# ziyaad30/ForwardTacotron

Hardware: AMD Instinct MI355X
Metric: mel_frames_per_sec_train_step (higher is better)
Workload: dtype f32

## Files before the change

### forwardtacotron_amd/csrc/ft_capi_core.hip

```cpp
#include <stdarg.h>
#include <stdio.h>
#include <string.h>

#include "../../include/fwdtaco_hip.h"
#include <mutex>
#include <utility>
#include <vector>

#include "ft_gemm.h"

static thread_local char g_err[512] = "";

void ft_set_error(const char* fmt, ...) {
  va_list ap;
  va_start(ap, fmt);
  vsnprintf(g_err, sizeof(g_err), fmt, ap);
  va_end(ap);
}

int ft_check_launch(const char* what) {
  hipError_t e = hipGetLastError();
  if (e != hipSuccess) {
    ft_set_error("%s: HIP launch failed: %s", what, hipGetErrorString(e));
    return FT_ERR_HIP;
// ... 455 lines not shown
static int conv1d_bwd_data_impl(const float* dy, long lddy, const float* wp, float* dx, long lddx, int B, int T, int Cin,
                                int Cout, int k, int Tbuf, int Tvalid, int accumulate, int wp_transposed,
                                const float* relu_mask, void* stream) {
  FT_REQUIRE(k >= 1 && Tvalid <= Tbuf, "conv1d_bwd_data: bad k/Tvalid");
  FtGemmBatch b;
  memset(&b, 0, sizeof(b));
  b.relu_mask = relu_mask;
  FtGemmTask& t = b.t[0];
  t.A = dy; t.B = wp; t.C = dx;
  t.lda = lddy; t.ldb = wp_transposed ? Cout : Cin; t.ldc = lddx; t.b_tap_stride = (long)Cout * Cin;
  t.M = B * T; t.N = Cin; t.K = Cout; t.taps = k;
  FtRowMap m = {T > 0 ? T : 1, Tbuf, 1, Tvalid, k / 2, -1};
  t.amap = m;
  t.accumulate = accumulate;
  return ft_launch_gemm_rows(&b, 1, !wp_transposed, (hipStream_t)stream);
}

static bool bank_bwd_partials(int B, int T, int Cin, int K) {
  const long tiles = (long)ft_cdiv((long)B * T, 128) * ft_cdiv(Cin, 128);
  return K >= 2 && Cin > 64 && (long)B * T > 64 && tiles < 192 && tiles * K >= 192;
}

size_t ft_conv_bank_bwd_data_workspace(int B, int T, int Cin, int K) {
  return bank_bwd_partials(B, T, Cin, K) ? (size_t)K * B * T * Cin * sizeof(float) : 0;
}

int ft_conv_bank_bwd_data(const float* dy, long lddy, const float* wp_all, float* dx, long lddx, int B, int T, int Cin,
                          int C, int K, int Tbuf, int wp_transposed, void* workspace, size_t workspace_bytes,
                          void* stream) {
  FT_REQUIRE(K >= 1 && K <= FT_MAX_TASKS, "conv_bank_bwd_data: K=%d unsupported (max %d)", K, FT_MAX_TASKS);
  FT_REQUIRE(Tbuf == T || Tbuf == T + 1, "conv_bank_bwd_data: Tbuf must be T or T+1");
  const bool partials = bank_bwd_partials(B, T, Cin, K);
  if (partials)
    FT_REQUIRE(workspace && workspace_bytes >= ft_conv_bank_bwd_data_workspace(B, T, Cin, K),
               "conv_bank_bwd_data: workspace too small");
  float* part = static_cast<float*>(workspace);
  FtGemmBatch b;
  memset(&b, 0, sizeof(b));
  long woff = 0;
  for (int i = 0; i < K; ++i) {
    const int k = i + 1;
    FtGemmTask& t = b.t[i];
    t.A = dy + (long)i * C; t.B = wp_all + woff;
    t.C = partials ? part + (long)i * B * T * Cin : dx;
    t.lda = lddy; t.ldb = wp_transposed ? C : Cin; t.ldc = partials ? Cin : lddx; t.b_tap_stride = (long)C * Cin;
    t.M = B * T; t.N = Cin; t.K = C; t.taps = k;
    const int Tvalid = (k % 2 == 0) ? Tbuf : T;
    FtRowMap m = {T > 0 ? T : 1, Tbuf, 1, Tvalid < Tbuf ? Tvalid : Tbuf, k / 2, -1};
    t.amap = m;
    woff += (long)k * C * Cin;
  }
  b.chain = partials ? 0 : K;
  if (partials && wp_transposed) {
    FtGemmBatch c = b;
    for (int i = 0; i < K; ++i) {
      c.t[i].C = dx;
      c.t[i].ldc = lddx;
    }
    c.chain = K;
    const size_t need = ft_rows_ksplit_floats(c, K, (hipStream_t)stream) * sizeof(float);
    if (need > 0 && need <= workspace_bytes) {
      c.ksplit_slab = part;
      return ft_launch_gemm_rows(&c, K, false, (hipStream_t)stream);
    }
  }
  int rc = ft_launch_gemm_rows(&b, K, !wp_transposed, (hipStream_t)stream);
  if (rc || !partials) return rc;
  return ft_launch_slab_sum(part, dx, B * T, Cin, K, lddx, (hipStream_t)stream);
}

static FtGemmTNTask conv_bw_task(const float* dy, long lddy, const float* x, long ldx, float* dw, int B, int T,
                                 int Cin, int Cout, int k, int Tbuf, int Tvalid) {
  FtGemmTNTask t;
  memset(&t, 0, sizeof(t));
  t.A = dy; t.B = x; t.dst = dw;
  t.lda = lddy; t.ldb = ldx;
// ... 151 lines not shown
```

### forwardtacotron_amd/csrc/ft_gemm.h

```cpp
#pragma once
#include "ft_common.h"

struct FtRowMap {
  int Tlog, bstride, tstride, Tvalid, shift0, shift_step;
};

static inline FtRowMap ft_rowmap_identity(int rows) {
  int n = rows > 0 ? rows : 1;
  FtRowMap m = {n, 0, 1, n, 0, 0};
  return m;
}
static inline FtRowMap ft_rowmap_layout(int rows, int tm_B) {
  if (tm_B <= 0) return ft_rowmap_identity(rows);
  int T = rows / tm_B;
  FtRowMap m = {T > 0 ? T : 1, 1, tm_B, T, 0, 0};
  return m;
}

struct FtGemmTask {
  const float* A;
  const float* B;
  float* C;
  const float* bias;
  const float* scale;
// ... 145 lines not shown
    int kk = 1, first = 0;
    while (first + kk <= q) {
      first += kk;
      ++kk;
    }
    w.kk = kk;
    w.zts = q - first;
    w.mtile = (kk - 1) * tpm + sub;
    w.s = blockIdx.z;
  } else {
    w.kk = 0;
    w.mtile = blockIdx.x;
    w.zts = blockIdx.z / S;
    w.s = blockIdx.z - w.zts * S;
  }
  return w;
}

static inline bool ft_rows_tile_is_big(long tiles128, int maxM, int maxN) { return tiles128 >= 192 && maxN > 64 && maxM > 64; }
static_assert(sizeof(FtGemmBatch) <= 4080, "FtGemmBatch travels as a kernel argument (4 KB limit)");
int ft_launch_gemm_rows(FtGemmBatch* batch, int ntasks, bool b_ncontig, hipStream_t stream);
size_t ft_rows_ksplit_floats(const FtGemmBatch& batch, int ntasks, hipStream_t stream);
int ft_launch_ksplit_reduce(const float* slab, int S, const FtGemmTask& t, hipStream_t stream);
bool ft_rows_b3p_ok(const FtGemmBatch& batch, int ntask);
int ft_launch_gemm_rows_b3(const FtGemmBatch& batch, bool big, dim3 grid, hipStream_t stream);
int ft_launch_gemm_tn_b3(const FtGemmTNTask& t, float* slab, int S, int rows_per_split, int tm, dim3 grid,
                         hipStream_t stream);
void ft_note_stream_slots(hipStream_t s, int slots);
int ft_stream_slots(hipStream_t s);
bool ft_gemm_b3_enabled();
int ft_gemm_precision();
int ft_launch_gemm_tn(const FtGemmTNTask& task, float* workspace, size_t workspace_floats,
                      hipStream_t stream);
size_t ft_gemm_tn_workspace_floats(const FtGemmTNTask& task);
int ft_launch_slab_sum(const float* slab, float* dst, int M, int N, int S, long ldm, hipStream_t stream);
```

### forwardtacotron_amd/csrc/ft_gemm.hip

```cpp
#include "ft_gemm.h"

namespace {

constexpr int BK = 32;

__device__ __forceinline__ float4 ld4(const float* p, int remaining, bool vec) {
  float4 v = make_float4(0.f, 0.f, 0.f, 0.f);
  if (remaining >= 4 && vec) {
    v = *reinterpret_cast<const float4*>(p);
  } else {
    if (remaining > 0) v.x = p[0];
    if (remaining > 1) v.y = p[1];
    if (remaining > 2) v.z = p[2];
    if (remaining > 3) v.w = p[3];
  }
  return v;
}

template <int TM, int TN, int LDA, int LDB>
__device__ __forceinline__ void mfma_stage(const float* ap, const float* bp, f32x16 (&acc)[TM][TN]) {
  float a0[TM], b0[TN], a1[TM], b1[TN];
#pragma unroll
  for (int i = 0; i < TM; ++i) a0[i] = ap[32 * i];
#pragma unroll
// ... 582 lines not shown
static int rows_ksplit_plan(const FtGemmBatch& b, int ntasks, hipStream_t stream) {
  static const bool enabled = [] {
    const char* e = getenv("FT_GEMM_KSPLIT");
    return !(e && e[0] == '0');
  }();
  const bool chained = b.chain > 1;
  if (!enabled || !(chained ? b.chain == ntasks : ntasks == 1) || !ft_gemm_b3_enabled()) return 1;
  const FtGemmTask& t0 = b.t[0];
  if (t0.nz > 1 || t0.relu || t0.scale || t0.stat || b.hw_mode || b.relu_mask || t0.N % 4 != 0 || t0.M <= 64 || t0.N <= 64) return 1;
  if (!ft_rows_b3p_ok(b, ntasks)) return 1;
  long stages = 0;
  for (int i = 0; i < ntasks; ++i) stages += (long)b.t[i].taps * ft_cdiv(b.t[i].K, 16);
  const long tiles = (long)ft_cdiv(t0.M, 128) * ft_cdiv(t0.N, 128);
  const long slots = ft_stream_slots(stream);
  if (stages < 128) return 1;
  long S = slots / (tiles > 0 ? tiles : 1);
  if (S > stages / 32) S = stages / 32;
  if (S > 16) S = 16;
  if (S < 2) return 1;
  const long per = (stages + S - 1) / S;
  return (int)((stages + per - 1) / per);
}

size_t ft_rows_ksplit_floats(const FtGemmBatch& batch, int ntasks, hipStream_t stream) {
  const int S = rows_ksplit_plan(batch, ntasks, stream);
  return S > 1 ? (size_t)S * batch.t[0].M * batch.t[0].N : 0;
}

int ft_launch_gemm_rows(FtGemmBatch* batch, int ntasks, bool b_ncontig, hipStream_t stream) {
  FT_REQUIRE(ntasks >= 1 && ntasks <= FT_MAX_TASKS, "gemm_rows: bad task count %d", ntasks);
  int maxM = 0, maxN = 0;
  long tiles128 = 0;
  for (int i = 0; i < ntasks; ++i) {
    FtGemmTask& t = batch->t[i];
    FT_REQUIRE(t.M >= 0 && t.N >= 0 && t.K >= 0 && t.taps >= 1, "gemm_rows: bad dims");
    FT_REQUIRE(t.amap.Tlog > 0, "gemm_rows: bad row map");
    if (t.cmap.Tlog <= 0) t.cmap = ft_rowmap_identity(t.M);
    if (t.nz <= 1) {
      t.nz = t.nz1 = 1;
      t.sA0 = t.sA1 = t.sB0 = t.sB1 = t.sC0 = t.sC1 = 0;
    }
    FT_REQUIRE(t.nz == 1 || ntasks == 1, "gemm_rows: strided batch needs a single task");
    FT_REQUIRE(t.nz1 >= 1 && t.nz % t.nz1 == 0, "gemm_rows: bad batch split");
    t.a_vec = (t.lda % 4 == 0) && (((uintptr_t)t.A) % 16 == 0) && (t.sA0 % 4 == 0) && (t.sA1 % 4 == 0);
    t.b_vec = (t.ldb % 4 == 0) && (t.b_tap_stride % 4 == 0) && (((uintptr_t)t.B) % 16 == 0) && (t.sB0 % 4 == 0) &&
              (t.sB1 % 4 == 0);
    if (t.M > maxM) maxM = t.M;
    if (t.N > maxN) maxN = t.N;
    tiles128 += (long)ft_cdiv(t.M, 128) * ft_cdiv(t.N, 128) * t.nz;
  }
  if (maxM == 0 || maxN == 0) return FT_OK;
  for (int i = ntasks; i < FT_MAX_TASKS; ++i) batch->t[i] = batch->t[0];
  const bool chained = batch->chain > 1;
  if (chained) {
    FT_REQUIRE(batch->chain == ntasks, "gemm_rows: chain must cover all tasks");
    for (int i = 0; i < ntasks; ++i)
      FT_REQUIRE(batch->t[i].M == batch->t[0].M && batch->t[i].N == batch->t[0].N && batch->t[i].nz == 1,
                 "gemm_rows: chained tasks must share M and N");
    tiles128 /= ntasks;
  } else {
    batch->chain = 0;
  }
  bool big = batch->force_tile ? batch->force_tile == 2 : ft_rows_tile_is_big(tiles128, maxM, maxN);
  batch->ksplit = 0;
  if (batch->ksplit_slab) {
    bool ok = !b_ncontig && ft_gemm_precision() == 0;
    for (int i = 0; i < ntasks && ok; ++i) {
      const FtGemmTask& t = batch->t[i];
      ok = (t.lda % 4 == 0) && (((uintptr_t)t.A) % 16 == 0) && (t.ldb % 4 == 0) && (t.b_tap_stride % 4 == 0) &&
           (((uintptr_t)t.B) % 16 == 0) && t.K % 4 == 0;
    }
    const int S = ok ? rows_ksplit_plan(*batch, ntasks, stream) : 1;
    if (S > 1) {
      batch->ksplit = S;
      big = true;
    }
  }
  const int bm = big ? 128 : 64;
  dim3 grid(ft_cdiv(maxM, bm), ft_cdiv(maxN, bm), chained ? 1 : (ntasks == 1 ? batch->t[0].nz : ntasks));
  if (batch->ksplit > 1) grid.z = batch->ksplit;
  FT_REQUIRE(grid.y <= 65535 && grid.z <= 65535, "gemm_rows: grid too large");
  bool fast = true;
  for (int i = 0; i < ntasks; ++i) {
    const FtGemmTask& t = batch->t[i];
    const bool k_ok = t.K % 4 == 0 || (b_ncontig && t.a_rowpad && t.lda >= ((t.K + 3) & ~3));
    fast = fast && t.a_vec && t.b_vec && k_ok && (!b_ncontig || t.N % 4 == 0);
  }
#define FT_ROWS_LAUNCH(TM_, BNC_)                                                                              \
  do {                                                                                                         \
    if (fast)                                                                                                  \
      hipLaunchKernelGGL((ft_gemm_rows_kernel<TM_, TM_, BNC_, true>), grid, dim3(256), 0, stream, *batch);     \
    else                                                                                                       \
      hipLaunchKernelGGL((ft_gemm_rows_kernel<TM_, TM_, BNC_, false>), grid, dim3(256), 0, stream, *batch);    \
  } while (0)
  GemmLog log;
  log.begin(stream);
  const bool b3 = fast && !b_ncontig && ((big && ft_gemm_b3_enabled()) || ft_gemm_precision() == 1);
  batch->stat_fused = b3 && big && !chained;
  if (b3) {
    (void)ft_launch_gemm_rows_b3(*batch, big, grid, stream);
  } else if (big) {
    if (b_ncontig) FT_ROWS_LAUNCH(2, true);
    else FT_ROWS_LAUNCH(2, false);
  } else {
    if (b_ncontig) FT_ROWS_LAUNCH(1, true);
    else FT_ROWS_LAUNCH(1, false);
  }
#undef FT_ROWS_LAUNCH
  if (GemmLog::on()) {
    double fl = 0;
    long sk = 0;
    for (int i = 0; i < ntasks; ++i) {
      const FtGemmTask& t = batch->t[i];
      fl += 2.0 * t.M * t.N * t.K * t.taps * t.nz;
      sk += (long)t.K * t.taps;
    }
    log.end(b_ncontig ? "rowsNN" : (b3 ? (ft_gemm_precision() == 1 ? "rowsBF" : "rowsB3") : "rowsNT"), maxM, maxN, sk, ntasks, batch->t[0].nz,
            big ? "128" : "64", fl);
  }
  int rc = ft_check_launch("gemm_rows");
  if (rc == FT_OK && batch->ksplit > 1) rc = ft_launch_ksplit_reduce(batch->ksplit_slab, batch->ksplit, batch->t[0], stream);
  return rc;
}

int ft_launch_slab_sum(const float* slab, float* dst, int M, int N, int S, long ldm, hipStream_t stream) {
  long total = (long)M * N;
  if (total == 0) return FT_OK;
  hipLaunchKernelGGL(ft_splitk_reduce_kernel, dim3(ft_cdiv(total, 256)), dim3(256), 0, stream, slab, dst, M, N, 1, S,
                     ldm, 1L, 0L, 0, 1, 1, 0L, 0L);
  return ft_check_launch("slab_sum");
}

int ft_launch_gemm_tn(const FtGemmTNTask& task_in, float* workspace, size_t workspace_floats,
                      hipStream_t stream) {
  FtGemmTNTask t = task_in;
  FT_REQUIRE(t.M >= 0 && t.N >= 0 && t.R >= 0 && t.taps >= 1, "gemm_tn: bad dims");
  if (t.M == 0 || t.N == 0) return FT_OK;
  if (t.nz <= 1) {
    t.nz = t.nz1 = 1;
    t.sA0 = t.sA1 = t.sB0 = t.sB1 = t.sD0 = t.sD1 = 0;
  }
// ... 62 lines not shown
```

### forwardtacotron_amd/csrc/ft_gemm_b3.hip

```cpp
#include "ft_gemm.h"
#include "ft_split.h"

namespace {

constexpr int BK = 32;
constexpr int RS = 104;

typedef __bf16 bf16x8 __attribute__((ext_vector_type(8)));
typedef unsigned short u16x4 __attribute__((ext_vector_type(4)));
typedef unsigned u32x4 __attribute__((ext_vector_type(4)));

__device__ __forceinline__ float4 ld4_sel(const float* p, const float* safe, bool ok) {
  const float4 v = *reinterpret_cast<const float4*>(ok ? p : safe);
  return ok ? v : make_float4(0.f, 0.f, 0.f, 0.f);
}

__device__ __forceinline__ unsigned rn_pack(float a, float b) { return ft_rn_pack(a, b); }
__device__ __forceinline__ void split_pair(float a, float b, unsigned& hi, unsigned& mid, unsigned& lo) {
  ft_split_pair(a, b, hi, mid, lo);
}
__device__ __forceinline__ void split3(const float4& v, u16x4& hi, u16x4& mid, u16x4& lo) {
  unsigned h[2], m[2], l[2];
  split_pair(v.x, v.y, h[0], m[0], l[0]);
  split_pair(v.z, v.w, h[1], m[1], l[1]);
  hi = __builtin_bit_cast(u16x4, uint2{h[0], h[1]});
  mid = __builtin_bit_cast(u16x4, uint2{m[0], m[1]});
  lo = __builtin_bit_cast(u16x4, uint2{l[0], l[1]});
}

__device__ __forceinline__ void store_split(unsigned short* row, const float4& v) {
  u16x4 h, m, l;
  split3(v, h, m, l);
  *reinterpret_cast<u16x4*>(row) = h;
  *reinterpret_cast<u16x4*>(row + 32) = m;
  *reinterpret_cast<u16x4*>(row + 64) = l;
}

__device__ __forceinline__ void store_rn(unsigned short* row, const float4& v) {
  typedef __bf16 bf16x4 __attribute__((ext_vector_type(4)));
  bf16x4 r = {(__bf16)v.x, (__bf16)v.y, (__bf16)v.z, (__bf16)v.w};
  *reinterpret_cast<bf16x4*>(row) = r;
}

template <int TM, int TN>
__device__ __forceinline__ void rows_b3_epilogue(const FtGemmTask& T, float* TC, f32x16 (&acc)[TM][TN], unsigned short* smem,
                                                 int m0, int n0, int tM, int tN, int tid, int mtile,
                                                 const float* relu_mask = nullptr) {
  const int wave = tid >> 6, lane = tid & 63;
  const int wm = wave >> 1, wn = wave & 1;
  const int half = lane >> 5, l31 = lane & 31;
  const float* ebias = T.bias;
  const float* escale = T.scale;
  const float* eshift = T.shift;
  const bool erelu = T.relu != 0, eacc = T.accumulate != 0;
  const long ldc = T.ldc, cbst = T.cmap.bstride, ctst = T.cmap.tstride;
  const int cTlog = T.cmap.Tlog;
  double* const stat = (TM == 2 && TN == 2) ? T.stat : nullptr;
  const int sTlog = T.amap.Tlog, sTv = T.stat_tvalid;
  const int srow0 = m0 + wm * 32 * TM + 4 * half;
  const int stb = stat ? srow0 % sTlog : 0;
  const bool ssmall = sTlog < 32 * TM;
  double* sred = reinterpret_cast<double*>(smem);
#pragma unroll
  for (int j = 0; j < TN; ++j) {
    const int col = n0 + wn * 32 * TN + 32 * j + l31;
    const bool col_ok = col < tN;
    const float bv = (ebias && col_ok) ? ebias[col] : 0.f;
// ... 21 lines not shown
          if (tt < sTv) {
            s0 += (double)v;
            s1 += (double)v * (double)v;
          }
        }
        if (escale) v = v * sc + sh;
        if (relu_mask && !(relu_mask[crow * ldc + col] > 0.f)) v = 0.f;
        if (eacc) v += *cp;
        *cp = v;
      }
    }
    if (stat) {
      s0 += __shfl_xor(s0, 32, 64);
      s1 += __shfl_xor(s1, 32, 64);
      if (half == 0) {
        double* q = sred + ((wm * 128) + wn * 32 * TN + 32 * j + l31) * 2;
        q[0] = s0;
        q[1] = s1;
      }
    }
  }
  if (stat) {
    __syncthreads();
    if (tid < 128 && n0 + tid < tN) {
      double* o = stat + ((long)mtile * T.stat_ld + T.stat_col0 + n0 + tid) * 2;
      o[0] = sred[tid * 2] + sred[(128 + tid) * 2];
      o[1] = sred[tid * 2 + 1] + sred[(128 + tid) * 2 + 1];
    }
  }
}

template <int TM, int TN, int NP>
__global__ __launch_bounds__(256, 2) void ft_gemm_rows_b3_kernel(FtGemmBatch batch) {
  const bool zbatch = batch.t[0].nz > 1;
  const FtGemmTask& T = batch.t[zbatch ? 0 : blockIdx.z];
  const float* TA = T.A;
  const float* TB = T.B;
  float* TC = T.C;
  if (zbatch) {
    const int z0 = blockIdx.z / T.nz1, z1 = blockIdx.z - z0 * T.nz1;
    TA += z0 * T.sA0 + z1 * T.sA1;
    TB += z0 * T.sB0 + z1 * T.sB1;
    TC += z0 * T.sC0 + z1 * T.sC1;
  }
  constexpr int BM = 64 * TM, BN = 64 * TN;
  constexpr int PA = BM / 32, PB = BN / 32;
  __shared__ __attribute__((aligned(16))) unsigned short smem[(BM + BN) * RS];
  unsigned short* As = smem;
  unsigned short* Bs = smem + BM * RS;

// ... 126 lines not shown
          constexpr int P1 = NP > 1 ? 1 : 0, P2 = NP - 1;
          acc[i][j] = __builtin_amdgcn_mfma_f32_32x32x16_bf16(a[i][0], b[j][P2], acc[i][j], 0, 0, 0);
          acc[i][j] = __builtin_amdgcn_mfma_f32_32x32x16_bf16(a[i][P1], b[j][P1], acc[i][j], 0, 0, 0);
          acc[i][j] = __builtin_amdgcn_mfma_f32_32x32x16_bf16(a[i][P1], b[j][0], acc[i][j], 0, 0, 0);
          acc[i][j] = __builtin_amdgcn_mfma_f32_32x32x16_bf16(a[i][0], b[j][P1], acc[i][j], 0, 0, 0);
          acc[i][j] = __builtin_amdgcn_mfma_f32_32x32x16_bf16(a[i][0], b[j][0], acc[i][j], 0, 0, 0);
        }
    }
    __syncthreads();
    if (c + 1 < nch) {
      store_stage();
      if (c + 2 < nch) load_stage();
      __syncthreads();
    }
  }

  if (batch.hw_mode) {
    ft_highway_epilogue<TM, TN>(batch, T, TC, acc, reinterpret_cast<float*>(smem), m0, n0, tid);
    return;
  }
  rows_b3_epilogue<TM, TN>(T, TC, acc, smem, m0, n0, tM, tN, tid, blockIdx.x, batch.relu_mask);
}

template <int NP>
__global__ __launch_bounds__(256, 2) void ft_gemm_rows_b3p_kernel(FtGemmBatch batch) {
  constexpr int TM = 2, TN = 2, BM = 128, BN = 128, SK = 16;
  constexpr int RW = NP == 3 ? 48 : 24;
  constexpr int BUF = (BM + BN) * RW;
  int bx, by;
  const int bz = blockIdx.z;
  {
    const int gy = gridDim.y;
    const int nwg = gridDim.x * gy;
    const int lin = blockIdx.x + gridDim.x * blockIdx.y;
    const int xcd = lin & 7, q = nwg >> 3, r = nwg & 7;
    const int w = (xcd < r ? xcd * (q + 1) : r * (q + 1) + (xcd - r) * q) + (lin >> 3);
    bx = w / gy;
    by = w - bx * gy;
  }
  const bool zbatch = batch.t[0].nz > 1;
  const int ksplit = batch.ksplit > 1 ? batch.ksplit : 1;
  const FtGemmTask& T = batch.t[(zbatch || ksplit > 1) ? 0 : bz];
  const float* TA = T.A;
  const float* TB = T.B;
  float* TC = T.C;
  if (zbatch) {
    const int z0 = bz / T.nz1, z1 = bz - z0 * T.nz1;
    TA += z0 * T.sA0 + z1 * T.sA1;
    TB += z0 * T.sB0 + z1 * T.sB1;
    TC += z0 * T.sC0 + z1 * T.sC1;
  }
  __shared__ __attribute__((aligned(16))) unsigned short smem[2 * BUF];

  const int m0 = bx * BM, n0 = by * BN;
  if (m0 >= T.M || n0 >= T.N) return;
  const int tid = threadIdx.x;
  const int h = tid & 1, rr = tid >> 1;

  const int tM = T.M, tN = T.N;
  const int nchain = batch.chain > 1 ? batch.chain : 1;
  constexpr unsigned OOB = 0x80000000u, NREC = 0x7fffffffu;
  int tK, taps, Tvalid, shift0, sstep, kch, a_t;
  long lda, btap, atst;
  const float* a_base;
  const float* b_base;
  bool a_ok;
  unsigned a_voff, vb, vbad0, vbad1;
  unsigned va0, va1, vb0, vb1;
  bool ktail;
  const float* tapA;
  const float* tapB;
  int l_task = 0, l_tap = 0, l_kc = 0;
  auto mask_tail = [&]() {
    va0 |= vbad0;
    va1 |= vbad1;
    vb0 |= vbad0;
    vb1 |= vbad1;
  };
  auto set_tap = [&]() {
    const int shift = shift0 + l_tap * sstep;
    const int ts = a_t + shift;
    va0 = (a_ok & (ts >= 0) & (ts < Tvalid)) ? a_voff : OOB;
    va1 = va0 + 32u;
    vb0 = vb;
    vb1 = vb + 32u;
    if (ktail && kch == 1) mask_tail();
    tapA = a_base + (long)shift * atst * lda;
    tapB = b_base + (long)l_tap * btap;
  };
  auto setup = [&](const FtGemmTask& S, const float* SA, const float* SB) {
    tK = S.K;
    taps = S.taps;
    lda = S.lda;
    btap = S.b_tap_stride;
    Tvalid = S.amap.Tvalid;
    shift0 = S.amap.shift0;
    sstep = S.amap.shift_step;
    atst = S.amap.tstride;
    kch = (tK + SK - 1) / SK;
    const int Tlog = S.amap.Tlog;
    const long abst = S.amap.bstride;
    const int bt0 = m0 / Tlog;
    long row0 = (long)bt0 * abst + (long)(m0 - bt0 * Tlog) * atst;
    if (m0 - bt0 * Tlog + BM > Tlog && (long)(bt0 + 1) * abst < row0)
      row0 = (long)(bt0 + 1) * abst;
    a_base = SA + row0 * lda;
    const int m = m0 + rr;
    a_ok = m < tM;
    const int b = m / Tlog;
    a_t = m - b * Tlog;
    a_voff = (unsigned)((((long)b * abst + (long)a_t * atst) - row0) * lda * 4) + 16u * h;
    b_base = SB + (long)n0 * S.ldb;
    vb = n0 + rr < tN ? (unsigned)((long)rr * S.ldb * 4) + 16u * h : OOB;
    const int kl = (kch - 1) * SK;
    ktail = tK % SK != 0;
    vbad0 = kl + 4 * h < tK ? 0u : OOB;
    vbad1 = kl + 8 + 4 * h < tK ? 0u : OOB;
    set_tap();
  };
  setup(T, TA, TB);
  int nch = 0;
  for (int i = 0; i < nchain; ++i) nch += batch.t[i].taps * ((batch.t[i].K + SK - 1) / SK);
  if (nchain == 1) nch = taps * kch;
  if (ksplit > 1) {
    const int per = (nch + ksplit - 1) / ksplit;
    int rem = bz * per;
    nch = nch - rem < per ? nch - rem : per;
    if (nch < 0) nch = 0;
    while (l_task < nchain - 1) {
      const int n = batch.t[l_task].taps * ((batch.t[l_task].K + SK - 1) / SK);
      if (rem < n) break;
      rem -= n;
      ++l_task;
    }
    if (l_task > 0) setup(batch.t[l_task], batch.t[l_task].A, batch.t[l_task].B);
    l_tap = rem / kch;
    l_kc = rem - l_tap * kch;
    set_tap();
    if (ktail && kch > 1 && l_kc == kch - 1) mask_tail();
  }

  struct Regs { u32x4 a0, a1, b0, b1, b2; };
  auto load_stage = [&](Regs& R) {
    auto uniform = [](const float* q) {
      const unsigned long long u = (unsigned long long)q;
      const unsigned lo = __builtin_amdgcn_readfirstlane((unsigned)u), hi = __builtin_amdgcn_readfirstlane((unsigned)(u >> 32));
      return reinterpret_cast<float*>(((unsigned long long)hi << 32) | lo);
    };
    const __amdgpu_buffer_rsrc_t rsA = __builtin_amdgcn_make_buffer_rsrc(uniform(tapA), 0, NREC, 0x00020000);
    const __amdgpu_buffer_rsrc_t rsB = __builtin_amdgcn_make_buffer_rsrc(uniform(tapB), 0, NREC, 0x00020000);
    const unsigned soff = (unsigned)__builtin_amdgcn_readfirstlane(l_kc * SK * 4);
    R.a0 = __builtin_amdgcn_raw_buffer_load_b128(rsA, va0, soff, 0);
    R.a1 = __builtin_amdgcn_raw_buffer_load_b128(rsA, va1, soff, 0);
    R.b0 = __builtin_amdgcn_raw_buffer_load_b128(rsB, vb0, soff, 0);
    R.b1 = __builtin_amdgcn_raw_buffer_load_b128(rsB, vb1, soff, 0);
    __builtin_amdgcn_sched_barrier(0);
  };
  auto advance = [&]() {
    if (++l_kc == kch) {
      l_kc = 0;
      if (++l_tap == taps) {
        l_tap = 0;
        if (++l_task < nchain) setup(batch.t[l_task], batch.t[l_task].A, batch.t[l_task].B);
      } else {
        set_tap();
      }
    } else if (ktail && l_kc == kch - 1) {
      mask_tail();
    }
  };
  auto put8 = [&](unsigned short* row, const u32x4& uu, const u32x4& vv) {
    const float4 u = __builtin_bit_cast(float4, uu), v = __builtin_bit_cast(float4, vv);
    if constexpr (NP == 1) {
      const uint4 w = make_uint4(rn_pack(u.x, u.y), rn_pack(u.z, u.w), rn_pack(v.x, v.y), rn_pack(v.z, v.w));
      *reinterpret_cast<uint4*>(row) = w;
    } else {
      unsigned hi[4], mid[4], lo[4];
      split_pair(u.x, u.y, hi[0], mid[0], lo[0]);
      split_pair(u.z, u.w, hi[1], mid[1], lo[1]);
      split_pair(v.x, v.y, hi[2], mid[2], lo[2]);
      split_pair(v.z, v.w, hi[3], mid[3], lo[3]);
      *reinterpret_cast<uint4*>(row) = make_uint4(hi[0], hi[1], hi[2], hi[3]);
      *reinterpret_cast<uint4*>(row + 16) = make_uint4(mid[0], mid[1], mid[2], mid[3]);
      *reinterpret_cast<uint4*>(row + 32) = make_uint4(lo[0], lo[1], lo[2], lo[3]);
    }
  };
  auto store_stage = [&](const Regs& R, unsigned short* buf) {
    put8(buf + rr * RW + 8 * h, R.a0, R.a1);
    put8(buf + (BM + rr) * RW + 8 * h, R.b0, R.b1);
  };

  const int wave = tid >> 6, lane = tid & 63;
  const int wm = wave >> 1, wn = wave & 1;
  const int half = lane >> 5, l31 = lane & 31;
  f32x16 acc[TM][TN];
#pragma unroll
  for (int i = 0; i < TM; ++i)
#pragma unroll
    for (int j = 0; j < TN; ++j)
#pragma unroll
      for (int e = 0; e < 16; ++e) acc[i][j][e] = 0.f;

  const int aoff = (wm * 64 + l31) * RW + 8 * half;
  const int boff = (BM + wn * 64 + l31) * RW + 8 * half;
  auto interleave = [&]() {
    __builtin_amdgcn_sched_group_barrier(0x100, 4 * NP, 0);
#pragma unroll
    for (int i = 0; i < TM * TN * (NP == 3 ? 6 : 1); ++i) {
      __builtin_amdgcn_sched_group_barrier(0x008, 1, 0);
      __builtin_amdgcn_sched_group_barrier(0x002, NP == 3 ? 5 : 8, 0);
    }
  };
  bf16x8 fa[TM][NP], fb[TN][NP], ga[TM][NP], gb[TN][NP];
  auto read_into = [&](bf16x8 (&xa)[TM][NP], bf16x8 (&xb)[TN][NP], const unsigned short* buf) {
#pragma unroll
    for (int i = 0; i < TM; ++i)
#pragma unroll
      for (int pl = 0; pl < NP; ++pl) xa[i][pl] = *reinterpret_cast<const bf16x8*>(buf + aoff + 32 * i * RW + 16 * pl);
#pragma unroll
    for (int j = 0; j < TN; ++j)
#pragma unroll
      for (int pl = 0; pl < NP; ++pl) xb[j][pl] = *reinterpret_cast<const bf16x8*>(buf + boff + 32 * j * RW + 16 * pl);
  };
  auto mfma_on = [&](bf16x8 (&xa)[TM][NP], bf16x8 (&xb)[TN][NP]) {
    constexpr int PA_[6] = {2, 0, 1, 1, 0, 0}, PB_[6] = {0, 2, 1, 0, 1, 0};
#pragma unroll
    for (int term = 0; term < (NP == 3 ? 6 : 1); ++term)
#pragma unroll
      for (int i = 0; i < TM; ++i)
#pragma unroll
        for (int j = 0; j < TN; ++j) {
          const int pa = NP == 3 ? PA_[term] : 0, pb = NP == 3 ? PB_[term] : 0;
          acc[i][j] = __builtin_amdgcn_mfma_f32_32x32x16_bf16(xa[i][pa], xb[j][pb], acc[i][j], 0, 0, 0);
// ... 66 lines not shown
    mfma_on(fa, fb);
  }
  }
  __syncthreads();
  if (ksplit > 1) {
    float* out = batch.ksplit_slab + (long)bz * tM * tN;
#pragma unroll
    for (int j = 0; j < TN; ++j) {
      const int col = n0 + wn * 32 * TN + 32 * j + l31;
#pragma unroll
      for (int i = 0; i < TM; ++i)
#pragma unroll
        for (int e = 0; e < 16; ++e) {
          const int row = m0 + wm * 32 * TM + 32 * i + (e & 3) + 8 * (e >> 2) + 4 * half;
          if (row < tM && col < tN) out[(long)row * tN + col] = acc[i][j][e];
        }
    }
    return;
  }
  if (batch.hw_mode) {
    ft_highway_epilogue<TM, TN>(batch, T, TC, acc, reinterpret_cast<float*>(smem), m0, n0, tid);
    return;
  }
  rows_b3_epilogue<TM, TN>(T, TC, acc, smem, m0, n0, tM, tN, tid, bx, batch.relu_mask);
}

__global__ __launch_bounds__(256) void ft_ksplit_reduce_kernel(const float* __restrict__ slab, int S, FtGemmTask T) {
  const long idx = ((long)blockIdx.x * 256 + threadIdx.x) * 4;
  const long total = (long)T.M * T.N;
  if (idx >= total) return;
  const int row = (int)(idx / T.N), col = (int)(idx - (long)row * T.N);
  float4 a = *reinterpret_cast<const float4*>(slab + idx);
  for (int z = 1; z < S; ++z) {
    const float4 v = *reinterpret_cast<const float4*>(slab + (long)z * total + idx);
    a.x += v.x; a.y += v.y; a.z += v.z; a.w += v.w;
  }
  if (T.bias) {
    a.x += T.bias[col]; a.y += T.bias[col + 1]; a.z += T.bias[col + 2]; a.w += T.bias[col + 3];
  }
  long crow = row;
  if (T.cmap.bstride != 0) {
    const int cb = row / T.cmap.Tlog;
    crow = (long)cb * T.cmap.bstride + (long)(row - cb * T.cmap.Tlog) * T.cmap.tstride;
  }
  float* cp = T.C + crow * T.ldc + col;
  if (T.accumulate) {
    a.x += cp[0]; a.y += cp[1]; a.z += cp[2]; a.w += cp[3];
// ... 475 lines not shown
    if (span_ok(t.amap, t.R, t.lda, t.taps) && span_ok(t.bmap, t.R, t.ldb, t.taps)) {
      if (bf16) hipLaunchKernelGGL((ft_gemm_tn_b3p_kernel<1>), grid, dim3(256), 0, stream, t, slab, S, rows_per_split);
      else hipLaunchKernelGGL((ft_gemm_tn_b3p_kernel<3>), grid, dim3(256), 0, stream, t, slab, S, rows_per_split);
      ++g_tn_pipelined;
      return FT_OK;
    }
  }
  if (tm == 2) {
    if (bf16) hipLaunchKernelGGL((ft_gemm_tn_b3_kernel<2, 2, 1>), grid, dim3(256), 0, stream, t, slab, S, rows_per_split);
    else hipLaunchKernelGGL((ft_gemm_tn_b3_kernel<2, 2, 3>), grid, dim3(256), 0, stream, t, slab, S, rows_per_split);
  } else {
    if (bf16) hipLaunchKernelGGL((ft_gemm_tn_b3_kernel<1, 1, 1>), grid, dim3(256), 0, stream, t, slab, S, rows_per_split);
    else hipLaunchKernelGGL((ft_gemm_tn_b3_kernel<1, 1, 3>), grid, dim3(256), 0, stream, t, slab, S, rows_per_split);
  }
  return FT_OK;
}

int ft_launch_ksplit_reduce(const float* slab, int S, const FtGemmTask& t, hipStream_t stream) {
  const long quads = ((long)t.M * t.N + 3) / 4;
  hipLaunchKernelGGL(ft_ksplit_reduce_kernel, dim3(ft_cdiv(quads, 256)), dim3(256), 0, stream, slab, S, t);
  return ft_check_launch("ksplit_reduce");
}

bool ft_rows_b3p_ok(const FtGemmBatch& batch, int ntask) {
  static const bool pipelined = [] {
    const char* e = getenv("FT_GEMM_PIPE");
    return !(e && e[0] == '0');
  }();
  bool span_ok = true;
  for (int i = 0; i < (batch.t[0].nz > 1 ? 1 : ntask) && i < FT_MAX_TASKS; ++i) {
    const FtGemmTask& t = batch.t[i];
    const long tl = t.amap.Tlog, ts = t.amap.tstride, bs = t.amap.bstride;
    const long rows = (tl < 128 ? tl : 128) * ts + (128 / tl + 2) * bs + tl * ts;
    span_ok = span_ok && ts >= 0 && bs >= 0 && rows * t.lda * 4 < (1L << 31) && 128L * t.ldb * 4 < (1L << 31);
  }
  return pipelined && span_ok;
}

int ft_launch_gemm_rows_b3(const FtGemmBatch& batch, bool big, dim3 grid, hipStream_t stream) {
  const bool bf16 = ft_gemm_precision() == 1;
  const int ntask = batch.chain > 1 ? batch.chain : (batch.ksplit > 1 ? 1 : (int)grid.z);
  const bool p_ok = ft_rows_b3p_ok(batch, ntask);
  FT_REQUIRE(batch.ksplit <= 1 || (big && p_ok), "gemm_rows: split-K planned for a launch the pipelined kernel cannot take");
  if (big && p_ok) {
    if (bf16) hipLaunchKernelGGL((ft_gemm_rows_b3p_kernel<1>), grid, dim3(256), 0, stream, batch);
    else hipLaunchKernelGGL((ft_gemm_rows_b3p_kernel<3>), grid, dim3(256), 0, stream, batch);
  } else if (big) {
    if (bf16) hipLaunchKernelGGL((ft_gemm_rows_b3_kernel<2, 2, 1>), grid, dim3(256), 0, stream, batch);
    else hipLaunchKernelGGL((ft_gemm_rows_b3_kernel<2, 2, 3>), grid, dim3(256), 0, stream, batch);
  } else {
    if (bf16) hipLaunchKernelGGL((ft_gemm_rows_b3_kernel<1, 1, 1>), grid, dim3(256), 0, stream, batch);
    else hipLaunchKernelGGL((ft_gemm_rows_b3_kernel<1, 1, 3>), grid, dim3(256), 0, stream, batch);
  }
  return FT_OK;
}
```

### lab/gemm_prod_lab.hip

```cpp
#include "../forwardtacotron_amd/csrc/ft_gemm_b3.hip"
#include <stdio.h>
#include <stdlib.h>
#include <string.h>
#include <vector>
int ft_gemm_precision() { return 0; }
int ft_fail(const char*, ...) { return -1; }

static void run(const char* name, const float* A, const float* B, float* C, int M, int N, int K) {
  FtGemmBatch batch;
  memset(&batch, 0, sizeof(batch));
  FtGemmTask& t = batch.t[0];
  t.A = A; t.B = B; t.C = C; t.lda = K; t.ldb = K; t.ldc = N; t.M = M; t.N = N; t.K = K; t.taps = 1;
  t.amap = ft_rowmap_identity(M); t.cmap = ft_rowmap_identity(M); t.nz = t.nz1 = 1; t.a_vec = t.b_vec = 1;
  for (int i = 1; i < FT_MAX_TASKS; ++i) batch.t[i] = batch.t[0];
  dim3 grid((M + 127) / 128, (N + 127) / 128, 1);
  hipEvent_t e0, e1;
  (void)hipEventCreate(&e0);
  (void)hipEventCreate(&e1);
  for (int i = 0; i < 3; ++i) ft_launch_gemm_rows_b3(batch, true, grid, 0);
  (void)hipEventRecord(e0);
  const int n = 10;
  for (int i = 0; i < n; ++i) ft_launch_gemm_rows_b3(batch, true, grid, 0);
  (void)hipEventRecord(e1);
  (void)hipEventSynchronize(e1);
  float ms;
  (void)hipEventElapsedTime(&ms, e0, e1);
  ms /= n;
  printf("%-30s M %d N %d K %d: %8.1f us  %6.1f TF(f32-eq)\n", name, M, N, K, ms * 1e3, 2.0 * M * N * K / ms / 1e9);
  fflush(stdout);
}

int main() {
  const int M = 27136, N = 2048, K = 1024;
  float *A, *B, *C;
  (void)hipMalloc(&A, (size_t)M * 4096 * 4);
  (void)hipMalloc(&B, (size_t)4096 * 4096 * 4);
  (void)hipMalloc(&C, (size_t)M * 4096 * 4);
  std::vector<float> h((size_t)M * 4096);
  srand(1);
  for (auto& v : h) v = (float)rand() / RAND_MAX * 2.f - 1.f;
  (void)hipMemcpy(A, h.data(), (size_t)M * 4096 * 4, hipMemcpyHostToDevice);
  (void)hipMemcpy(B, h.data(), (size_t)4096 * 4096 * 4, hipMemcpyHostToDevice);
  const char* e = getenv("FT_GEMM_PIPE");
  run(e && e[0] == '0' ? "product two-barrier" : "product pipelined", A, B, C, M, N, K);
  run("same, M = 26912", A, B, C, 26912, N, K);
  run("K = 512", A, B, C, 26912, N, 512);
  run("N = 512, K = 4096", A, B, C, 26912, 512, 4096);
  run("N = 4096, K = 512", A, B, C, 26912, 4096, 512);
  return 0;
}
```

Measured before the change: 947,200.

## Add 256-row tile variant of pipelined GEMM for tall narrow products

Templates the pipelined rows GEMM kernel on tile height and adds a 256x128 tile with 512 threads. Each B tile fetched from memory is then reused across twice as many rows. A heuristic enables it for tall, narrow, deep single products (M>=8192, N<=512, enough K stages and tiles). The load/store staging, masking and stat epilogue are adapted for the taller tile. Separately, the conv-bank backward-data path now sizes a workspace and tries split-K whenever a workspace exists, not only when partials are chosen. The gains come with a risk of lower occupancy and fewer blocks on the GPU.

Measured after the change: 946,400 (median of 4 runs). About the same (-0.1%).

```diff
diff --git a/forwardtacotron_amd/csrc/ft_capi_core.hip b/forwardtacotron_amd/csrc/ft_capi_core.hip
--- a/forwardtacotron_amd/csrc/ft_capi_core.hip
+++ b/forwardtacotron_amd/csrc/ft_capi_core.hip
@@ -501,7 +501,11 @@
 }
 
 size_t ft_conv_bank_bwd_data_workspace(int B, int T, int Cin, int K) {
-  return bank_bwd_partials(B, T, Cin, K) ? (size_t)K * B * T * Cin * sizeof(float) : 0;
+  if (bank_bwd_partials(B, T, Cin, K)) return (size_t)K * B * T * Cin * sizeof(float);
+  const long tiles = (long)ft_cdiv((long)B * T, 128) * ft_cdiv(Cin, 128);
+  long S = tiles > 0 ? 512 / tiles : 0;
+  if (S > 16) S = 16;
+  return K >= 2 && S >= 2 ? (size_t)S * B * T * Cin * sizeof(float) : 0;
 }
 
 int ft_conv_bank_bwd_data(const float* dy, long lddy, const float* wp_all, float* dx, long lddx, int B, int T, int Cin,
@@ -530,7 +534,7 @@
     woff += (long)k * C * Cin;
   }
   b.chain = partials ? 0 : K;
-  if (partials && wp_transposed) {
+  if (wp_transposed && workspace) {
     FtGemmBatch c = b;
     for (int i = 0; i < K; ++i) {
       c.t[i].C = dx;
diff --git a/forwardtacotron_amd/csrc/ft_gemm.h b/forwardtacotron_amd/csrc/ft_gemm.h
--- a/forwardtacotron_amd/csrc/ft_gemm.h
+++ b/forwardtacotron_amd/csrc/ft_gemm.h
@@ -191,8 +191,8 @@
 int ft_launch_gemm_rows(FtGemmBatch* batch, int ntasks, bool b_ncontig, hipStream_t stream);
 size_t ft_rows_ksplit_floats(const FtGemmBatch& batch, int ntasks, hipStream_t stream);
 int ft_launch_ksplit_reduce(const float* slab, int S, const FtGemmTask& t, hipStream_t stream);
-bool ft_rows_b3p_ok(const FtGemmBatch& batch, int ntask);
-int ft_launch_gemm_rows_b3(const FtGemmBatch& batch, bool big, dim3 grid, hipStream_t stream);
+bool ft_rows_b3p_ok(const FtGemmBatch& batch, int ntask, int bm = 128);
+int ft_launch_gemm_rows_b3(const FtGemmBatch& batch, bool big, bool tall, dim3 grid, hipStream_t stream);
 int ft_launch_gemm_tn_b3(const FtGemmTNTask& t, float* slab, int S, int rows_per_split, int tm, dim3 grid,
                          hipStream_t stream);
 void ft_note_stream_slots(hipStream_t s, int slots);
diff --git a/forwardtacotron_amd/csrc/ft_gemm.hip b/forwardtacotron_amd/csrc/ft_gemm.hip
--- a/forwardtacotron_amd/csrc/ft_gemm.hip
+++ b/forwardtacotron_amd/csrc/ft_gemm.hip
@@ -628,6 +628,23 @@
   return (int)((stages + per - 1) / per);
 }
 
+static bool rows_use_bm256(const FtGemmBatch& b, int ntasks, int maxM, int maxN, long tiles256, hipStream_t stream) {
+  static const int mode = [] {
+    const char* e = getenv("FT_GEMM_BM256");
+    return e && e[0] == '0' ? 0 : (e && e[0] == '2' ? 2 : 1);
+  }();
+  if (mode == 0 || ft_gemm_precision() != 0 || b.ksplit > 1 || !ft_rows_b3p_ok(b, ntasks, 256)) return false;
+  if (mode == 2) return true;
+  long stages = 0;
+  for (int i = 0; i < ntasks; ++i) {
+    const long st = (long)b.t[i].taps * ft_cdiv(b.t[i].K, 16);
+    stages = b.chain > 1 ? stages + st : (st > stages ? st : stages);
+  }
+  const long cus = ft_stream_slots(stream) / 2;
+  const bool one_product = ntasks == 1 || b.chain > 1;
+  return one_product && maxM >= 8192 && maxN <= 512 && stages >= 16 && tiles256 * 4 >= cus * 3;
+}
+
 size_t ft_rows_ksplit_floats(const FtGemmBatch& batch, int ntasks, hipStream_t stream) {
   const int S = rows_ksplit_plan(batch, ntasks, stream);
   return S > 1 ? (size_t)S * batch.t[0].M * batch.t[0].N : 0;
@@ -636,7 +653,7 @@
 int ft_launch_gemm_rows(FtGemmBatch* batch, int ntasks, bool b_ncontig, hipStream_t stream) {
   FT_REQUIRE(ntasks >= 1 && ntasks <= FT_MAX_TASKS, "gemm_rows: bad task count %d", ntasks);
   int maxM = 0, maxN = 0;
-  long tiles128 = 0;
+  long tiles128 = 0, tiles256 = 0;
   for (int i = 0; i < ntasks; ++i) {
     FtGemmTask& t = batch->t[i];
     FT_REQUIRE(t.M >= 0 && t.N >= 0 && t.K >= 0 && t.taps >= 1, "gemm_rows: bad dims");
@@ -654,6 +671,7 @@
     if (t.M > maxM) maxM = t.M;
     if (t.N > maxN) maxN = t.N;
     tiles128 += (long)ft_cdiv(t.M, 128) * ft_cdiv(t.N, 128) * t.nz;
+    tiles256 += (long)ft_cdiv(t.M, 256) * ft_cdiv(t.N, 128) * t.nz;
   }
   if (maxM == 0 || maxN == 0) return FT_OK;
   for (int i = ntasks; i < FT_MAX_TASKS; ++i) batch->t[i] = batch->t[0];
@@ -664,6 +682,7 @@
       FT_REQUIRE(batch->t[i].M == batch->t[0].M && batch->t[i].N == batch->t[0].N && batch->t[i].nz == 1,
                  "gemm_rows: chained tasks must share M and N");
     tiles128 /= ntasks;
+    tiles256 /= ntasks;
   } else {
     batch->chain = 0;
   }
@@ -682,16 +701,18 @@
       big = true;
     }
   }
-  const int bm = big ? 128 : 64;
-  dim3 grid(ft_cdiv(maxM, bm), ft_cdiv(maxN, bm), chained ? 1 : (ntasks == 1 ? batch->t[0].nz : ntasks));
-  if (batch->ksplit > 1) grid.z = batch->ksplit;
-  FT_REQUIRE(grid.y <= 65535 && grid.z <= 65535, "gemm_rows: grid too large");
   bool fast = true;
   for (int i = 0; i < ntasks; ++i) {
     const FtGemmTask& t = batch->t[i];
     const bool k_ok = t.K % 4 == 0 || (b_ncontig && t.a_rowpad && t.lda >= ((t.K + 3) & ~3));
     fast = fast && t.a_vec && t.b_vec && k_ok && (!b_ncontig || t.N % 4 == 0);
   }
+  const bool b3 = fast && !b_ncontig && ((big && ft_gemm_b3_enabled()) || ft_gemm_precision() == 1);
+  const bool tall = b3 && big && rows_use_bm256(*batch, ntasks, maxM, maxN, tiles256, stream);
+  const int bm = big ? 128 : 64;
+  dim3 grid(ft_cdiv(maxM, tall ? 256 : bm), ft_cdiv(maxN, bm), chained ? 1 : (ntasks == 1 ? batch->t[0].nz : ntasks));
+  if (batch->ksplit > 1) grid.z = batch->ksplit;
+  FT_REQUIRE(grid.y <= 65535 && grid.z <= 65535, "gemm_rows: grid too large");
 #define FT_ROWS_LAUNCH(TM_, BNC_)                                                                              \
   do {                                                                                                         \
     if (fast)                                                                                                  \
@@ -701,10 +722,9 @@
   } while (0)
   GemmLog log;
   log.begin(stream);
-  const bool b3 = fast && !b_ncontig && ((big && ft_gemm_b3_enabled()) || ft_gemm_precision() == 1);
   batch->stat_fused = b3 && big && !chained;
   if (b3) {
-    (void)ft_launch_gemm_rows_b3(*batch, big, grid, stream);
+    (void)ft_launch_gemm_rows_b3(*batch, big, tall, grid, stream);
   } else if (big) {
     if (b_ncontig) FT_ROWS_LAUNCH(2, true);
     else FT_ROWS_LAUNCH(2, false);
@@ -722,7 +742,7 @@
       sk += (long)t.K * t.taps;
     }
     log.end(b_ncontig ? "rowsNN" : (b3 ? (ft_gemm_precision() == 1 ? "rowsBF" : "rowsB3") : "rowsNT"), maxM, maxN, sk, ntasks, batch->t[0].nz,
-            big ? "128" : "64", fl);
+            tall ? "256" : (big ? "128" : "64"), fl);
   }
   int rc = ft_check_launch("gemm_rows");
   if (rc == FT_OK && batch->ksplit > 1) rc = ft_launch_ksplit_reduce(batch->ksplit_slab, batch->ksplit, batch->t[0], stream);
diff --git a/forwardtacotron_amd/csrc/ft_gemm_b3.hip b/forwardtacotron_amd/csrc/ft_gemm_b3.hip
--- a/forwardtacotron_amd/csrc/ft_gemm_b3.hip
+++ b/forwardtacotron_amd/csrc/ft_gemm_b3.hip
@@ -42,7 +42,7 @@
   *reinterpret_cast<bf16x4*>(row) = r;
 }
 
-template <int TM, int TN>
+template <int TM, int TN, int WM = 2>
 __device__ __forceinline__ void rows_b3_epilogue(const FtGemmTask& T, float* TC, f32x16 (&acc)[TM][TN], unsigned short* smem,
                                                  int m0, int n0, int tM, int tN, int tid, int mtile,
                                                  const float* relu_mask = nullptr) {
@@ -110,10 +110,12 @@
   }
   if (stat) {
     __syncthreads();
-    if (tid < 128 && n0 + tid < tN) {
-      double* o = stat + ((long)mtile * T.stat_ld + T.stat_col0 + n0 + tid) * 2;
-      o[0] = sred[tid * 2] + sred[(128 + tid) * 2];
-      o[1] = sred[tid * 2 + 1] + sred[(128 + tid) * 2 + 1];
+    const int sub = tid >> 7, c = tid & 127;
+    if (sub < WM / 2 && n0 + c < tN && m0 + 128 * sub < tM) {
+      double* o = stat + ((long)(mtile * (WM / 2) + sub) * T.stat_ld + T.stat_col0 + n0 + c) * 2;
+      const double* q = sred + (2 * sub * 128 + c) * 2;
+      o[0] = q[0] + q[256];
+      o[1] = q[1] + q[257];
     }
   }
 }
@@ -286,9 +288,11 @@
   rows_b3_epilogue<TM, TN>(T, TC, acc, smem, m0, n0, tM, tN, tid, blockIdx.x, batch.relu_mask);
 }
 
-template <int NP>
-__global__ __launch_bounds__(256, 2) void ft_gemm_rows_b3p_kernel(FtGemmBatch batch) {
-  constexpr int TM = 2, TN = 2, BM = 128, BN = 128, SK = 16;
+template <int NP, int BM>
+__global__ __launch_bounds__(2 * BM, 2) void ft_gemm_rows_b3p_kernel(FtGemmBatch batch) {
+  static_assert(BM == 128 || BM == 256, "rows_b3p: 128- or 256-row tiles");
+  constexpr int TM = 2, TN = 2, BN = 128, SK = 16;
+  constexpr bool TALL = BM == 256;
   constexpr int RW = NP == 3 ? 48 : 24;
   constexpr int BUF = (BM + BN) * RW;
   int bx, by;
@@ -319,33 +323,46 @@
   const int m0 = bx * BM, n0 = by * BN;
   if (m0 >= T.M || n0 >= T.N) return;
   const int tid = threadIdx.x;
-  const int h = tid & 1, rr = tid >> 1;
+  const int h = TALL ? tid & 3 : tid & 1, rr = TALL ? tid >> 2 : tid >> 1;
+  const int qpos = TALL ? 4 * (((h & 1) << 1) | (h >> 1)) : 8 * h;
 
   const int tM = T.M, tN = T.N;
   const int nchain = batch.chain > 1 ? batch.chain : 1;
   constexpr unsigned OOB = 0x80000000u, NREC = 0x7fffffffu;
-  int tK, taps, Tvalid, shift0, sstep, kch, a_t;
+  int tK, taps, Tvalid, shift0, sstep, kch, a_t, a_t2;
   long lda, btap, atst;
   const float* a_base;
   const float* b_base;
   bool a_ok;
-  unsigned a_voff, vb, vbad0, vbad1;
+  unsigned a_voff, a_voff2, vb, vbad0, vbad1;
   unsigned va0, va1, vb0, vb1;
   bool ktail;
   const float* tapA;
   const float* tapB;
   int l_task = 0, l_tap = 0, l_kc = 0;
   auto mask_tail = [&]() {
-    va0 |= vbad0;
-    va1 |= vbad1;
-    vb0 |= vbad0;
-    vb1 |= vbad1;
+    if constexpr (TALL) {
+      va0 |= vbad0;
+      va1 |= vbad0;
+      vb0 |= vbad0;
+    } else {
+      va0 |= vbad0;
+      va1 |= vbad1;
+      vb0 |= vbad0;
+      vb1 |= vbad1;
+    }
   };
   auto set_tap = [&]() {
     const int shift = shift0 + l_tap * sstep;
     const int ts = a_t + shift;
-    va0 = (a_ok & (ts >= 0) & (ts < Tvalid)) ? a_voff : OOB;
-    va1 = va0 + 32u;
+    if constexpr (TALL) {
+      const int ts2 = a_t2 + shift;
+      va0 = (unsigned)ts < (unsigned)Tvalid ? a_voff : OOB;
+      va1 = (unsigned)ts2 < (unsigned)Tvalid ? a_voff2 : OOB;
+    } else {
+      va0 = (a_ok & (ts >= 0) & (ts < Tvalid)) ? a_voff : OOB;
+      va1 = va0 + 32u;
+    }
     vb0 = vb;
     vb1 = vb + 32u;
     if (ktail && kch == 1) mask_tail();
@@ -374,6 +391,14 @@
     const int b = m / Tlog;
     a_t = m - b * Tlog;
     a_voff = (unsigned)((((long)b * abst + (long)a_t * atst) - row0) * lda * 4) + 16u * h;
+    if constexpr (TALL) {
+      const int m2 = m + 128;
+      const int b2 = m2 / Tlog;
+      a_t2 = m2 - b2 * Tlog;
+      a_voff2 = (unsigned)((((long)b2 * abst + (long)a_t2 * atst) - row0) * lda * 4) + 16u * h;
+      if (!a_ok) a_t = -(1 << 30);
+      if (m2 >= tM) a_t2 = -(1 << 30);
+    }
     b_base = SB + (long)n0 * S.ldb;
     vb = n0 + rr < tN ? (unsigned)((long)rr * S.ldb * 4) + 16u * h : OOB;
     const int kl = (kch - 1) * SK;
@@ -417,7 +442,7 @@
     R.a0 = __builtin_amdgcn_raw_buffer_load_b128(rsA, va0, soff, 0);
     R.a1 = __builtin_amdgcn_raw_buffer_load_b128(rsA, va1, soff, 0);
     R.b0 = __builtin_amdgcn_raw_buffer_load_b128(rsB, vb0, soff, 0);
-    R.b1 = __builtin_amdgcn_raw_buffer_load_b128(rsB, vb1, soff, 0);
+    if constexpr (!TALL) R.b1 = __builtin_amdgcn_raw_buffer_load_b128(rsB, vb1, soff, 0);
     __builtin_amdgcn_sched_barrier(0);
   };
   auto advance = [&]() {
@@ -449,9 +474,28 @@
       *reinterpret_cast<uint4*>(row + 32) = make_uint4(lo[0], lo[1], lo[2], lo[3]);
     }
   };
+  auto put4 = [&](unsigned short* row, const u32x4& uu) {
+    const float4 u = __builtin_bit_cast(float4, uu);
+    if constexpr (NP == 1) {
+      *reinterpret_cast<uint2*>(row) = make_uint2(rn_pack(u.x, u.y), rn_pack(u.z, u.w));
+    } else {
+      unsigned hi[2], mid[2], lo[2];
+      split_pair(u.x, u.y, hi[0], mid[0], lo[0]);
+      split_pair(u.z, u.w, hi[1], mid[1], lo[1]);
+      *reinterpret_cast<uint2*>(row) = make_uint2(hi[0], hi[1]);
+      *reinterpret_cast<uint2*>(row + 16) = make_uint2(mid[0], mid[1]);
+      *reinterpret_cast<uint2*>(row + 32) = make_uint2(lo[0], lo[1]);
+    }
+  };
   auto store_stage = [&](const Regs& R, unsigned short* buf) {
-    put8(buf + rr * RW + 8 * h, R.a0, R.a1);
-    put8(buf + (BM + rr) * RW + 8 * h, R.b0, R.b1);
+    if constexpr (TALL) {
+      put4(buf + rr * RW + qpos, R.a0);
+      put4(buf + (128 + rr) * RW + qpos, R.a1);
+      put4(buf + (BM + rr) * RW + qpos, R.b0);
+    } else {
+      put8(buf + rr * RW + qpos, R.a0, R.a1);
+      put8(buf + (BM + rr) * RW + qpos, R.b0, R.b1);
+    }
   };
 
   const int wave = tid >> 6, lane = tid & 63;
@@ -472,7 +516,7 @@
 #pragma unroll
     for (int i = 0; i < TM * TN * (NP == 3 ? 6 : 1); ++i) {
       __builtin_amdgcn_sched_group_barrier(0x008, 1, 0);
-      __builtin_amdgcn_sched_group_barrier(0x002, NP == 3 ? 5 : 8, 0);
+      __builtin_amdgcn_sched_group_barrier(0x002, NP == 3 ? (TALL ? 4 : 5) : (TALL ? 6 : 8), 0);
     }
   };
   bf16x8 fa[TM][NP], fb[TN][NP], ga[TM][NP], gb[TN][NP];
@@ -585,7 +629,7 @@
     ft_highway_epilogue<TM, TN>(batch, T, TC, acc, reinterpret_cast<float*>(smem), m0, n0, tid);
     return;
   }
-  rows_b3_epilogue<TM, TN>(T, TC, acc, smem, m0, n0, tM, tN, tid, bx, batch.relu_mask);
+  rows_b3_epilogue<TM, TN, BM / 64>(T, TC, acc, smem, m0, n0, tM, tN, tid, bx, batch.relu_mask);
 }
 
 __global__ __launch_bounds__(256) void ft_ksplit_reduce_kernel(const float* __restrict__ slab, int S, FtGemmTask T) {
@@ -1107,7 +1151,7 @@
   return ft_check_launch("ksplit_reduce");
 }
 
-bool ft_rows_b3p_ok(const FtGemmBatch& batch, int ntask) {
+bool ft_rows_b3p_ok(const FtGemmBatch& batch, int ntask, int bm) {
   static const bool pipelined = [] {
     const char* e = getenv("FT_GEMM_PIPE");
     return !(e && e[0] == '0');
@@ -1116,20 +1160,24 @@
   for (int i = 0; i < (batch.t[0].nz > 1 ? 1 : ntask) && i < FT_MAX_TASKS; ++i) {
     const FtGemmTask& t = batch.t[i];
     const long tl = t.amap.Tlog, ts = t.amap.tstride, bs = t.amap.bstride;
-    const long rows = (tl < 128 ? tl : 128) * ts + (128 / tl + 2) * bs + tl * ts;
+    const long rows = (tl < bm ? tl : bm) * ts + (bm / tl + 2) * bs + tl * ts;
     span_ok = span_ok && ts >= 0 && bs >= 0 && rows * t.lda * 4 < (1L << 31) && 128L * t.ldb * 4 < (1L << 31);
   }
   return pipelined && span_ok;
 }
 
-int ft_launch_gemm_rows_b3(const FtGemmBatch& batch, bool big, dim3 grid, hipStream_t stream) {
+int ft_launch_gemm_rows_b3(const FtGemmBatch& batch, bool big, bool tall, dim3 grid, hipStream_t stream) {
   const bool bf16 = ft_gemm_precision() == 1;
   const int ntask = batch.chain > 1 ? batch.chain : (batch.ksplit > 1 ? 1 : (int)grid.z);
-  const bool p_ok = ft_rows_b3p_ok(batch, ntask);
-  FT_REQUIRE(batch.ksplit <= 1 || (big && p_ok), "gemm_rows: split-K planned for a launch the pipelined kernel cannot take");
-  if (big && p_ok) {
-    if (bf16) hipLaunchKernelGGL((ft_gemm_rows_b3p_kernel<1>), grid, dim3(256), 0, stream, batch);
-    else hipLaunchKernelGGL((ft_gemm_rows_b3p_kernel<3>), grid, dim3(256), 0, stream, batch);
+  const bool p_ok = ft_rows_b3p_ok(batch, ntask, tall ? 256 : 128);
+  FT_REQUIRE(batch.ksplit <= 1 || (big && p_ok && !tall), "gemm_rows: split-K planned for a launch the pipelined kernel cannot take");
+  FT_REQUIRE(!tall || (big && p_ok), "gemm_rows: 256-row tile planned for a launch the pipelined kernel cannot take");
+  if (tall) {
+    if (bf16) hipLaunchKernelGGL((ft_gemm_rows_b3p_kernel<1, 256>), grid, dim3(512), 0, stream, batch);
+    else hipLaunchKernelGGL((ft_gemm_rows_b3p_kernel<3, 256>), grid, dim3(512), 0, stream, batch);
+  } else if (big && p_ok) {
+    if (bf16) hipLaunchKernelGGL((ft_gemm_rows_b3p_kernel<1, 128>), grid, dim3(256), 0, stream, batch);
+    else hipLaunchKernelGGL((ft_gemm_rows_b3p_kernel<3, 128>), grid, dim3(256), 0, stream, batch);
   } else if (big) {
     if (bf16) hipLaunchKernelGGL((ft_gemm_rows_b3_kernel<2, 2, 1>), grid, dim3(256), 0, stream, batch);
     else hipLaunchKernelGGL((ft_gemm_rows_b3_kernel<2, 2, 3>), grid, dim3(256), 0, stream, batch);
diff --git a/lab/gemm_prod_lab.hip b/lab/gemm_prod_lab.hip
--- a/lab/gemm_prod_lab.hip
+++ b/lab/gemm_prod_lab.hip
@@ -5,41 +5,48 @@
 #include <vector>
 int ft_gemm_precision() { return 0; }
 int ft_fail(const char*, ...) { return -1; }
+void ft_set_error(const char* fmt, ...) { fprintf(stderr, "error: %s\n", fmt); }
+int ft_check_launch(const char*) { return hipGetLastError() == hipSuccess ? 0 : -1; }
 
-static void run(const char* name, const float* A, const float* B, float* C, int M, int N, int K) {
+static void run(const char* name, const float* A, const float* B, float* C, int M, int N, int K, bool tall = false) {
   FtGemmBatch batch;
   memset(&batch, 0, sizeof(batch));
   FtGemmTask& t = batch.t[0];
   t.A = A; t.B = B; t.C = C; t.lda = K; t.ldb = K; t.ldc = N; t.M = M; t.N = N; t.K = K; t.taps = 1;
   t.amap = ft_rowmap_identity(M); t.cmap = ft_rowmap_identity(M); t.nz = t.nz1 = 1; t.a_vec = t.b_vec = 1;
   for (int i = 1; i < FT_MAX_TASKS; ++i) batch.t[i] = batch.t[0];
-  dim3 grid((M + 127) / 128, (N + 127) / 128, 1);
+  dim3 grid((M + (tall ? 255 : 127)) / (tall ? 256 : 128), (N + 127) / 128, 1);
   hipEvent_t e0, e1;
   (void)hipEventCreate(&e0);
   (void)hipEventCreate(&e1);
-  for (int i = 0; i < 3; ++i) ft_launch_gemm_rows_b3(batch, true, grid, 0);
+  for (int i = 0; i < 3; ++i) ft_launch_gemm_rows_b3(batch, true, tall, grid, 0);
   (void)hipEventRecord(e0);
   const int n = 10;
-  for (int i = 0; i < n; ++i) ft_launch_gemm_rows_b3(batch, true, grid, 0);
+  for (int i = 0; i < n; ++i) ft_launch_gemm_rows_b3(batch, true, tall, grid, 0);
   (void)hipEventRecord(e1);
   (void)hipEventSynchronize(e1);
   float ms;
   (void)hipEventElapsedTime(&ms, e0, e1);
   ms /= n;
-  printf("%-30s M %d N %d K %d: %8.1f us  %6.1f TF(f32-eq)\n", name, M, N, K, ms * 1e3, 2.0 * M * N * K / ms / 1e9);
+  printf("%-30s %s M %d N %d K %d: %8.1f us  %6.1f TF(f32-eq)\n", name, tall ? "256x128" : "128x128", M, N, K, ms * 1e3,
+         2.0 * M * N * K / ms / 1e9);
   fflush(stdout);
 }
 
 int main() {
   const int M = 27136, N = 2048, K = 1024;
   float *A, *B, *C;
-  (void)hipMalloc(&A, (size_t)M * 4096 * 4);
+  const size_t a_floats = (size_t)M * 9216;
+  (void)hipMalloc(&A, a_floats * 4);
   (void)hipMalloc(&B, (size_t)4096 * 4096 * 4);
   (void)hipMalloc(&C, (size_t)M * 4096 * 4);
   std::vector<float> h((size_t)M * 4096);
   srand(1);
   for (auto& v : h) v = (float)rand() / RAND_MAX * 2.f - 1.f;
-  (void)hipMemcpy(A, h.data(), (size_t)M * 4096 * 4, hipMemcpyHostToDevice);
+  for (size_t off = 0; off < a_floats; off += h.size()) {
+    const size_t n = a_floats - off < h.size() ? a_floats - off : h.size();
+    (void)hipMemcpy(A + off, h.data(), n * 4, hipMemcpyHostToDevice);
+  }
   (void)hipMemcpy(B, h.data(), (size_t)4096 * 4096 * 4, hipMemcpyHostToDevice);
   const char* e = getenv("FT_GEMM_PIPE");
   run(e && e[0] == '0' ? "product two-barrier" : "product pipelined", A, B, C, M, N, K);
@@ -47,5 +54,11 @@
   run("K = 512", A, B, C, 26912, N, 512);
   run("N = 512, K = 4096", A, B, C, 26912, 512, 4096);
   run("N = 4096, K = 512", A, B, C, 26912, 4096, 512);
+  const int shapes[][3] = {{26944, 256, 6144}, {26944, 2048, 768}, {26944, 256, 1536}, {26944, 256, 512},
+                           {26944, 512, 256}, {26944, 1536, 256}, {26944, 80, 9216}, {26944, 80, 1024}};
+  for (const auto& sh : shapes) {
+    run("frame", A, B, C, sh[0], sh[1], sh[2], false);
+    run("frame", A, B, C, sh[0], sh[1], sh[2], true);
+  }
   return 0;
 }
```
